# HazyResearch/hyena-dna

Hardware: AMD Instinct MI355X
Metric: nucleotides/sec fwd+bwd at L=1M d=256; fftconv achieved HBM GB/s vs peak (higher is better)
Workload: dtype f32

## Files before the change

### hyena_dna_amd/_lib.py

```python
import ctypes
import os
import threading

import torch

HERE = os.path.dirname(os.path.abspath(__file__))
LIB_PATH = os.path.join(HERE, "csrc", "libhyena_fftconv.so")
ABI_VERSION = 3

HYENA_F32, HYENA_BF16, HYENA_F16 = 0, 1, 2
MAX_L = 1048576
PLAN_NONE, PLAN_ONCHIP, PLAN_TWO_LEVEL = 0, 1, 2

_DTYPES = {torch.float32: HYENA_F32, torch.bfloat16: HYENA_BF16, torch.float16: HYENA_F16}

_lock = threading.Lock()
_lib = None
_tables = {}
_workspace = {}


class HyenaLibraryError(RuntimeError):
    pass

# ... 503 lines not shown
def fftconv_fwd(u, k, bias, chunk=None, save=False, grad=None):
    _require_gpu(u, "u")
    B, D, L = u.shape
    u, k = as_rows(u), as_rows(k)
    ldx, ldk = ld_of(u), ld_of(k)
    out = empty_like_rows(u)
    if B == 0:
        return (out, torch.empty(0, dtype=torch.uint8, device=u.device)) if save else out
    chunk = _chunk_override() if chunk is None else int(chunk)
    tables = tables_for(u.device, L)
    nbytes = lib().hyena_fftconv_workspace_bytes(B, D, L, 0, chunk)
    if (save or torch.is_grad_enabled()) if grad is None else grad:
        nbytes = max(nbytes, lib().hyena_fftconv_workspace_bytes(B, D, L, 1, chunk))
    ws, stream = workspace_for(u.device, nbytes)
    bp = bias.data_ptr() if bias is not None else None
    with _backend.guard(u.device):
        saved = torch.empty(saved_bytes(B, D, L), dtype=torch.uint8, device=u.device) if save else None
        check(lib().hyena_fftconv_fwd_ld(u.data_ptr(), k.data_ptr(), bp, out.data_ptr(), B, D, L, ldx, ldk, dtype_code(u.dtype),
                                         tables.data_ptr(), ws.data_ptr(), ws.numel(), chunk,
                                         saved.data_ptr() if save else None, saved.numel() if save else 0, stream))
    return (out, saved) if save else out


def _same_pitch(t, ld):
    if ld_of(t) == ld:
        return t
    r = empty_rows(t.shape[:-1], t.shape[-1], t.dtype, t.device, pitch=ld)
    r.copy_(t)
    return r


def fftconv_bwd(dout, u, k, bias, need_du=True, need_dk=True, chunk=None, saved=None):
    _require_gpu(dout, "dout")
    B, D, L = dout.shape
    dout = as_rows(dout)
    ldx = ld_of(dout)
    if u is not None:
        u = _same_pitch(as_rows(u), ldx)
    if k is not None:
        k = as_rows(k)
    ldk = ld_of(k) if k is not None else row_pitch(L)
    du = empty_like_rows(dout) if need_du else None
    dk = empty_rows((D,), L, torch.float32, dout.device, pitch=ldk) if need_dk else None
    dbias = torch.empty((D,), dtype=torch.float32, device=dout.device) if need_dk else None
    if B == 0:
        return du, None if dk is None else dk.zero_(), None if dbias is None else dbias.zero_()
    chunk = _chunk_override() if chunk is None else int(chunk)
    tables = tables_for(dout.device, L)
    nbytes = lib().hyena_fftconv_workspace_bytes(B, D, L, 1, chunk)
    ws, stream = workspace_for(dout.device, nbytes)
    bp = bias.data_ptr() if bias is not None else None
    ptr = lambda t: t.data_ptr() if t is not None else None
    with _backend.guard(dout.device):
        check(lib().hyena_fftconv_bwd_ld(dout.data_ptr(), ptr(u), None if saved is not None else ptr(k), bp, ptr(du), ptr(dk), ptr(dbias),
                                         B, D, L, ldx, ldk, dtype_code(dout.dtype), tables.data_ptr(), ws.data_ptr(), ws.numel(),
                                         chunk, ptr(saved), saved.numel() if saved is not None else 0, stream))
    return du, dk, dbias


def mixer_pre_fwd(x, w, b, L):
    _require_gpu(x, "x")
    B, Lx, D3 = x.shape
    D = D3 // 3
    vg = torch.empty((B, D, L), dtype=x.dtype, device=x.device)
    with _backend.guard(x.device):
        check(lib().hyena_mixer_pre_fwd(x.data_ptr(), w.data_ptr(), b.data_ptr(), vg.data_ptr(), B, L, Lx, D,
                                        dtype_code(x.dtype), _backend.stream(x.device)))
    return vg


def mixer_post_fwd(y, x, w, b):
    _require_gpu(x, "x")
    B, D, L = y.shape
    z = torch.empty((B, L, D), dtype=x.dtype, device=x.device)
    with _backend.guard(x.device):
        check(lib().hyena_mixer_post_fwd(y.data_ptr(), x.data_ptr(), w.data_ptr(), b.data_ptr(), z.data_ptr(), B, L,
                                         x.shape[1], D, dtype_code(x.dtype), _backend.stream(x.device)))
    return z


def mixer_partials(x, L):
    B, Lx, D3 = x.shape
    n = lib().hyena_mixer_partial_floats(B, L, D3 // 3)
    return torch.empty(n, dtype=torch.float32, device=x.device).view(B, -1, D3, 4)


def mixer_post_bwd(dz, y, x, w, b, dx, part):
    B, D, L = y.shape
    dy = torch.empty_like(y)
    with _backend.guard(x.device):
        check(lib().hyena_mixer_post_bwd(dz.data_ptr(), y.data_ptr(), x.data_ptr(), w.data_ptr(), b.data_ptr(),
                                         dy.data_ptr(), dx.data_ptr(), part.data_ptr(), B, L, x.shape[1], D,
                                         dtype_code(x.dtype), _backend.stream(x.device)))
    return dy


def mixer_pre_bwd(dvg, x, w, b, dx, part):
    B, D, L = dvg.shape
    with _backend.guard(x.device):
        check(lib().hyena_mixer_pre_bwd(dvg.data_ptr(), x.data_ptr(), w.data_ptr(), b.data_ptr(), dx.data_ptr(),
                                        part.data_ptr(), B, L, x.shape[1], D, dtype_code(x.dtype),
                                        _backend.stream(x.device)))


def cm_pre_fwd(xT, bin_, w, b, L):
    _require_gpu(xT, "xT")
    D3, B, Lx = xT.shape
# ... 643 lines not shown
```

### hyena_dna_amd/csrc/fftconv.hip

```cpp
#include "fftconv_kernels.h"
#include "mixer_kernels.h"
#include "filter_kernels.h"
#include "block_kernels.h"
#include "../../include/hyena_fftconv.h"
#include "../../include/hyena_mixer.h"
#include "../../include/hyena_filter.h"
#include "../../include/hyena_block.h"

#include <cmath>
#include <cstdio>
#include <cstdlib>
#include <vector>

using namespace hyena;

#include "launch.h"
#include "onchip_host.h"

namespace {

struct Plan {
    int L, M, M1;
    int R;
};
// ... 245 lines not shown
        if (hipMemcpyAsync(d_tables, h.data(), h.size() * sizeof(c32), hipMemcpyHostToDevice, (hipStream_t)stream) != hipSuccess)
            return HYENA_ERR_LAUNCH;
        if (hipStreamSynchronize((hipStream_t)stream) != hipSuccess) return HYENA_ERR_LAUNCH;
#endif
        return HYENA_OK;
    }
    const double tau = 6.283185307179586476925286766559;
    for (int i = 0; i < 1024; ++i) {
        double a = -tau * (double)i / (double)p.M;
        h[i].x = (float)std::cos(a);
        h[i].y = (float)std::sin(a);
        double r = -tau * (double)i / 1024.0;
        h[2048 + i].x = (float)std::cos(r);
        h[2048 + i].y = (float)std::sin(r);
    }
    for (int s = 0; s < 32; ++s)
        for (int j = 0; j < 32; ++j) {
            double r = -tau * (double)(s * j) / 1024.0;
            h[3072 + s * 32 + j].x = (float)std::cos(r);
            h[3072 + s * 32 + j].y = (float)std::sin(r);
        }
    for (int i = 0; i < p.M1; ++i) {
        double a = -tau * (double)i / (double)p.M1;
        h[1024 + i].x = (float)std::cos(a);
        h[1024 + i].y = (float)std::sin(a);
    }
#ifdef HIPEMU
    memcpy(d_tables, h.data(), h.size() * sizeof(c32));
#else
    if (hipMemcpyAsync(d_tables, h.data(), h.size() * sizeof(c32), hipMemcpyHostToDevice, (hipStream_t)stream) != hipSuccess)
        return HYENA_ERR_LAUNCH;
    if (hipStreamSynchronize((hipStream_t)stream) != hipSuccess) return HYENA_ERR_LAUNCH;
#endif
    return HYENA_OK;
}

int hyena_fftconv_default_chunk(int B, int D, int L, int backward) {
    Plan p;
    if (!make_plan(L, &p) || B < 1 || D < 1) return 0;
    if (p.R) return D;
    const size_t per_channel = (size_t)(backward ? 2 * B + 2 : B + 1) * p.M * sizeof(c32);
    size_t c = CACHE_BUDGET / per_channel;
    const size_t cmax = ((size_t)1 << 28) / p.M;
    if (c > cmax) c = cmax;
    if (c < 1) c = 1;
    if (c > (size_t)D) c = D;
    return (int)c;
}

size_t hyena_fftconv_workspace_bytes(int B, int D, int L, int backward, int chunk) {
    Plan p;
    if (!make_plan(L, &p) || B < 1 || D < 1) return 0;
    if (p.R)
        return oc::spectrum_bytes(D, p.R) + (backward ? oc::dk_partial_bytes(p.R, B, D, L) + (oc::dk1_ok(p.R, B) ? oc::spectrum_bytes(D, p.R) : 0) : 0);
    if (chunk <= 0) chunk = hyena_fftconv_default_chunk(B, D, L, backward);
    if (chunk > D) chunk = D;
    if ((size_t)chunk * p.M > ((size_t)1 << 28)) chunk = (int)(((size_t)1 << 28) / p.M);
    return (size_t)(backward ? 2 * B + 2 : B + 1) * chunk * p.M * sizeof(c32) +
           (backward ? (size_t)B * chunk * 2 * 1024 * sizeof(c32) : 0);
}

static inline c32* saved_wk(void* saved) { return reinterpret_cast<c32*>(saved); }
static inline c32* saved_wu(void* saved, int D, int M) { return reinterpret_cast<c32*>(saved) + (size_t)D * M; }

size_t hyena_fftconv_saved_bytes(int B, int D, int L) {
    Plan p;
    if (!make_plan(L, &p) || B < 1 || D < 1) return 0;
    if (p.R) return oc::spectrum_bytes(D, p.R);
    return (size_t)(B + 1) * D * p.M * sizeof(c32);
}

static int fwd_impl(const void* u, const float* k, const float* bias, void* out, int B, int D, int L, int ldx, int ldk, int dtype,
                    const void* d_tables, void* workspace, size_t workspace_bytes, int chunk, void* saved,
                    size_t saved_bytes, void* stream) {
    Plan p;
    if (u == nullptr || k == nullptr || out == nullptr || d_tables == nullptr || workspace == nullptr || B < 1 ||
        D < 1 || ldx < L || ldk < L || (dtype != HYENA_F32 && dtype != HYENA_BF16 && dtype != HYENA_F16))
        return HYENA_ERR_BAD_ARG;
    const oc::Pitch ld = {ldx, ldk};
    if (!make_plan(L, &p)) return HYENA_ERR_UNSUPPORTED_L;
    if (p.R) {
        if ((size_t)D * p.M * sizeof(c32) >= ((size_t)1 << 32)) return HYENA_ERR_BAD_ARG;
        if (workspace_bytes < oc::spectrum_bytes(D, p.R)) return HYENA_ERR_WORKSPACE;
        if (saved != nullptr && saved_bytes < oc::spectrum_bytes(D, p.R)) return HYENA_ERR_WORKSPACE;
        if (oc::small_ok(p.R, B, D, L, ld, dtype))
            return oc::launch_small_fwd(p.R, u, out, k, bias, saved, d_tables, B, D, L, ld, dtype, stream);
        void* H = saved ? saved : workspace;
        int st = oc::launch_spec(p.R, k, bias, H, d_tables, D, L, ld, stream);
        if (st) return st;
        return oc::launch_conv(p.R, u, out, H, d_tables, B, D, L, ld, dtype, 0, stream);
    }
    if (chunk <= 0) chunk = hyena_fftconv_default_chunk(B, D, L, 0);
    if (chunk > D) chunk = D;
    if ((size_t)chunk * p.M > ((size_t)1 << 28)) chunk = (int)(((size_t)1 << 28) / p.M);
    if (workspace_bytes < hyena_fftconv_workspace_bytes(B, D, L, 0, chunk)) return HYENA_ERR_WORKSPACE;
    if (saved != nullptr && saved_bytes < hyena_fftconv_saved_bytes(B, D, L)) return HYENA_ERR_WORKSPACE;

    const Tables tab = tables_from(d_tables);
    c32* wsWk = reinterpret_cast<c32*>(workspace);
    c32* wsW = wsWk + (size_t)chunk * p.M;
    const size_t es = elem_size(dtype);
    int st;
    for (int d0 = 0; d0 < D; d0 += chunk) {
        const int cd = (D - d0 < chunk) ? D - d0 : chunk;
        c32* Wk = saved ? saved_wk(saved) + (size_t)d0 * p.M : wsWk;
        c32* Wu = saved ? saved_wu(saved, D, p.M) + (size_t)d0 * p.M : wsW;
        const int ub = saved ? D : cd;
        ColArgs ck;
        ck.x = k + (size_t)d0 * ldk; ck.W = Wk; ck.tab = tab; ck.L = L; ck.inner = cd; ck.w_bstride = cd;
        ck.outer_stride = 0; ck.inner_stride = ldk; ck.aux0 = nullptr; ck.x2 = nullptr; ck.W2 = nullptr;
        if ((st = launch_col<false>(HYENA_F32, p.M1, ck, cd, stream))) return st;
        ColArgs cu;
        cu.x = reinterpret_cast<const char*>(u) + (size_t)d0 * ldx * es; cu.W = Wu; cu.tab = tab; cu.L = L; cu.inner = cd;
        cu.w_bstride = ub;
        cu.outer_stride = (long)D * ldx; cu.inner_stride = ldx; cu.aux0 = nullptr; cu.x2 = nullptr; cu.W2 = nullptr;
        if ((st = launch_col<false>(dtype, p.M1, cu, B * cd, stream))) return st;
        RowArgs rc;
        rc.X = Wu; rc.U = Wk; rc.S = nullptr; rc.S0 = nullptr; rc.bias = bias ? bias + d0 : nullptr; rc.K = nullptr; rc.Y = wsW;
        rc.x_bstride = ub; rc.u_bstride = 0; rc.y_bstride = cd; rc.tab = tab;
        rc.M1 = p.M1; rc.inner = cd; rc.B = B; rc.scale = 1.0f / (float)p.M;
        if ((st = launch_row_prod2<MODE_CONV>(rc, stream))) return st;
        ColArgs co = cu;
        co.x = reinterpret_cast<char*>(out) + (size_t)d0 * ldx * es; co.W = wsW; co.w_bstride = cd;
        if ((st = launch_col<true>(dtype, p.M1, co, B * cd, stream))) return st;
    }
    return HYENA_OK;
}

static int bwd_impl(const void* dout, const void* u, const float* k, const float* bias, void* du, float* dk,
                    float* dbias, int B, int D, int L, int ldx, int ldk, int dtype, const void* d_tables, void* workspace,
                    size_t workspace_bytes, int chunk, const void* saved_c, size_t saved_bytes, void* stream) {
    Plan p;
    void* saved = const_cast<void*>(saved_c);
    const oc::Pitch ld = {ldx, ldk};
    if (dout == nullptr || (u == nullptr && saved == nullptr) || (k == nullptr && saved == nullptr) ||
        d_tables == nullptr || workspace == nullptr || B < 1 || D < 1 || ldx < L || ldk < L ||
        (dtype != HYENA_F32 && dtype != HYENA_BF16 && dtype != HYENA_F16))
        return HYENA_ERR_BAD_ARG;
    if (dbias != nullptr && dk == nullptr) return HYENA_ERR_BAD_ARG;
    if (!make_plan(L, &p)) return HYENA_ERR_UNSUPPORTED_L;
    if (p.R) {
        if (dk != nullptr && u == nullptr) return HYENA_ERR_BAD_ARG;
        if (p.R == 1 && (size_t)B * D * ldx * elem_size(dtype) >= ((size_t)1 << 32)) return HYENA_ERR_BAD_ARG;
        if ((size_t)D * p.M * sizeof(c32) >= ((size_t)1 << 32)) return HYENA_ERR_BAD_ARG;
        if (workspace_bytes < hyena_fftconv_workspace_bytes(B, D, L, 1, chunk)) return HYENA_ERR_WORKSPACE;
        if (saved != nullptr && saved_bytes < oc::spectrum_bytes(D, p.R)) return HYENA_ERR_WORKSPACE;
        void* partials = reinterpret_cast<char*>(workspace) + oc::spectrum_bytes(D, p.R);
        int st;
        if ((du != nullptr || dk != nullptr) && oc::small_ok(p.R, B, D, L, ld, dtype)) {
            const void* H = saved;
            if (H == nullptr) {
                if ((st = oc::launch_small_fwd(p.R, nullptr, nullptr, k, bias, workspace, d_tables, 0, D, L, ld, dtype, stream))) return st;
                H = workspace;
            }
            return oc::launch_small_bwd(p.R, dout, u, du, dk, dbias, H, d_tables, B, D, L, ld, dtype, stream);
        }
        if (du != nullptr) {
            const void* H = saved;
            if (H == nullptr) {
                if ((st = oc::launch_spec(p.R, k, bias, workspace, d_tables, D, L, ld, stream))) return st;
                H = workspace;
            }
            if (dk != nullptr && oc::dkdu_ok(p.R, B))
                return oc::launch_dkdu(p.R, dout, u, du, H, dk, dbias, partials, d_tables, B, D, L, ld, dtype, stream);
            if ((st = oc::launch_conv(p.R, dout, du, H, d_tables, B, D, L, ld, dtype, 1, stream))) return st;
        }
        if (dk != nullptr && oc::dk1_ok(p.R, B)) {
            void* uspec = reinterpret_cast<char*>(partials) + oc::dk_partial_bytes(p.R, B, D, L);
            return oc::launch_dk1(p.R, dout, u, dk, dbias, uspec, d_tables, D, L, ld, dtype, stream);
        }
        if (dk != nullptr && (st = oc::launch_dk(p.R, dout, u, dk, dbias, partials, d_tables, B, D, L, ld, dtype, stream))) return st;
        return HYENA_OK;
    }
    if (chunk <= 0) chunk = hyena_fftconv_default_chunk(B, D, L, 1);
    if (chunk > D) chunk = D;
    if ((size_t)chunk * p.M > ((size_t)1 << 28)) chunk = (int)(((size_t)1 << 28) / p.M);
    if (workspace_bytes < hyena_fftconv_workspace_bytes(B, D, L, 1, chunk)) return HYENA_ERR_WORKSPACE;
    if (saved != nullptr && saved_bytes < hyena_fftconv_saved_bytes(B, D, L)) return HYENA_ERR_WORKSPACE;

    const Tables tab = tables_from(d_tables);
    c32* wsWk = reinterpret_cast<c32*>(workspace);
    c32* Sdk = wsWk + (size_t)chunk * p.M;
    c32* Wg = Sdk + (size_t)chunk * p.M;
    c32* wsWu = Wg + (size_t)B * chunk * p.M;
    c32* S0 = wsWu + (size_t)B * chunk * p.M;
    const size_t es = elem_size(dtype);
    int st;
    for (int d0 = 0; d0 < D; d0 += chunk) {
        const int cd = (D - d0 < chunk) ? D - d0 : chunk;
        c32* Wk = saved ? saved_wk(saved) + (size_t)d0 * p.M : wsWk;
        c32* Wu = saved ? saved_wu(saved, D, p.M) + (size_t)d0 * p.M : wsWu;
        const int ub = saved ? D : cd;
        ColArgs cg;
        cg.x = reinterpret_cast<const char*>(dout) + (size_t)d0 * ldx * es; cg.W = Wg; cg.tab = tab; cg.L = L; cg.inner = cd;
        cg.w_bstride = cd;
        cg.outer_stride = (long)D * ldx; cg.inner_stride = ldx; cg.aux0 = nullptr; cg.x2 = nullptr; cg.W2 = nullptr;
        ColArgs cgu = cg;
        if (dk != nullptr && !saved) { cgu.x2 = reinterpret_cast<const char*>(u) + (size_t)d0 * ldx * es; cgu.W2 = Wu; }
        if ((st = launch_col<false>(dtype, p.M1, cgu, B * cd, stream))) return st;
        ColArgs ck;
        ck.x = saved ? nullptr : k + (size_t)d0 * ldk; ck.W = Wk; ck.tab = tab; ck.L = L; ck.inner = cd; ck.w_bstride = cd;
        ck.outer_stride = 0; ck.inner_stride = ldk; ck.aux0 = nullptr; ck.x2 = nullptr; ck.W2 = nullptr;
        if (du != nullptr && !saved && (st = launch_col<false>(HYENA_F32, p.M1, ck, cd, stream))) return st;
        RowArgs rb;
        rb.X = Wg; rb.U = Wu; rb.S = Sdk; rb.S0 = S0; rb.bias = bias ? bias + d0 : nullptr; rb.K = Wk; rb.Y = Wg;
        rb.x_bstride = cd; rb.u_bstride = ub; rb.y_bstride = cd; rb.tab = tab;
        rb.M1 = p.M1; rb.inner = cd; rb.B = B; rb.scale = 1.0f / (float)p.M;
        if (dk != nullptr) {
            if (du != nullptr) st = launch_row_bwd<true>(rb, stream);
            else st = launch_row_bwd<false>(rb, stream);
            if (st) return st;
            ColArgs cdk;
            cdk.x = dk + (size_t)d0 * ldk; cdk.W = Sdk; cdk.tab = tab; cdk.L = L; cdk.inner = cd; cdk.w_bstride = cd;
            cdk.outer_stride = 0; cdk.inner_stride = ldk; cdk.aux0 = dbias ? dbias + d0 : nullptr; cdk.x2 = nullptr; cdk.W2 = nullptr;
            if ((st = launch_col<true>(HYENA_F32, p.M1, cdk, cd, stream))) return st;
        } else {
// ... 599 lines not shown
```

### hyena_dna_amd/csrc/onchip_dk.hip

```cpp
#define HY_PACKED_F32 1
#ifndef OC_X1_HALVES
#define OC_X1_HALVES 0
#endif
#include <cstdlib>
#include "onchip_kernels.h"
#include "launch.h"
#include "onchip_host.h"
#include "../../include/hyena_fftconv.h"

namespace hyena {
namespace oc {

template <int R, int NP, bool HALF>
static int dk_rh(const DkArgs& a, void* stream) {
    typedef DkCfg<R, NP> K;
    static thread_local int done = -1;
    hy_allow_lds(dk_kernel<R, NP, HALF, 0>, K::LDS, &done);
    HY_LAUNCH((dk_kernel<R, NP, HALF, 0>), dim3(a.D, a.S), dim3(K::WGT), K::LDS, stream, a);
    if constexpr (NP == 2) {
        static thread_local int done1 = -1;
        hy_allow_lds(dk_kernel<R, NP, HALF, 1>, K::LDS, &done1);
        HY_LAUNCH((dk_kernel<R, NP, HALF, 1>), dim3(a.D, a.S), dim3(K::WGT), K::LDS, stream, a);
    }
    if (a.S > 1) HY_LAUNCH((dk_sum_kernel<0>), dim3((a.L + 255) / 256, a.D), dim3(256), 0, stream, a);
    return hy_launch_error() ? HYENA_ERR_LAUNCH : HYENA_OK;
}
template <int R, int NP>
static int dk_r(const DkArgs& a, void* stream) {
    return a.dtype == DT_F32 ? dk_rh<R, NP, false>(a, stream) : dk_rh<R, NP, true>(a, stream);
}
template <int R, bool HALF>
static int dkdu_rh(const DkArgs& a, void* stream) {
    typedef DkCfg<R, 1> K;
    static thread_local int done = -1;
    hy_allow_lds((dk_kernel<R, 1, HALF, 0, true>), K::LDS, &done);
    HY_LAUNCH((dk_kernel<R, 1, HALF, 0, true>), dim3(a.D, a.S), dim3(K::WGT), K::LDS, stream, a);
    if (a.S > 1) HY_LAUNCH((dk_sum_kernel<0>), dim3((a.L + 255) / 256, a.D), dim3(256), 0, stream, a);
    return hy_launch_error() ? HYENA_ERR_LAUNCH : HYENA_OK;
}
template <int R>
static int dkdu_r(const DkArgs& a, void* stream) {
    return a.dtype == DT_F32 ? dkdu_rh<R, false>(a, stream) : dkdu_rh<R, true>(a, stream);
}

template <int R, bool HALF>
static int small_fwd_rh(const SmallFwdArgs& a, void* stream) {
    typedef SmallCfg<R> S;
    static thread_local int done = -1;
    hy_allow_lds(small_fwd_kernel<R, HALF>, S::LDS_FWD, &done);
    HY_LAUNCH((small_fwd_kernel<R, HALF>), dim3(a.D, 1), dim3(S::WGT_FWD), S::LDS_FWD, stream, a);
    return hy_launch_error() ? HYENA_ERR_LAUNCH : HYENA_OK;
}
template <int R, bool HALF>
static int small_bwd_rh(const SmallBwdArgs& a, void* stream) {
    typedef SmallCfg<R> S;
    static thread_local int done = -1;
    hy_allow_lds(small_bwd_kernel<R, HALF>, S::LDS_BWD, &done);
    HY_LAUNCH((small_bwd_kernel<R, HALF>), dim3(a.D), dim3(S::WGT_BWD), S::LDS_BWD, stream, a);
    return hy_launch_error() ? HYENA_ERR_LAUNCH : HYENA_OK;
}
int launch_small_fwd(int R, const void* x, void* out, const float* k, const float* bias, void* Hout, const void* tab, int B, int D, int L,
                     Pitch ld, int dtype, void* stream) {
    SmallFwdArgs a;
    a.x = x; a.out = out; a.k = k; a.bias = bias; a.Hout = reinterpret_cast<c32*>(Hout); a.tab = reinterpret_cast<const c32*>(tab);
    a.B = B; a.D = D; a.L = L; a.dtype = dtype; a.ldx = ld.ldx; a.ldk = ld.ldk;
    const bool half = dtype != DT_F32;
    if (R == 1) return half ? small_fwd_rh<1, true>(a, stream) : small_fwd_rh<1, false>(a, stream);
    if (R == 2) return half ? small_fwd_rh<2, true>(a, stream) : small_fwd_rh<2, false>(a, stream);
    return HYENA_ERR_UNSUPPORTED_L;
}
int launch_small_bwd(int R, const void* dout, const void* u, void* du, float* dk, float* dbias, const void* H, const void* tab, int B, int D,
                     int L, Pitch ld, int dtype, void* stream) {
    SmallBwdArgs a;
    a.dout = dout; a.u = u; a.du = du; a.dk = dk; a.dbias = dbias; a.H = reinterpret_cast<const c32*>(H);
    a.tab = reinterpret_cast<const c32*>(tab); a.B = B; a.D = D; a.L = L; a.dtype = dtype; a.ldx = ld.ldx; a.ldk = ld.ldk;
    const bool half = dtype != DT_F32;
    if (R == 1) return half ? small_bwd_rh<1, true>(a, stream) : small_bwd_rh<1, false>(a, stream);
    if (R == 2) return half ? small_bwd_rh<2, true>(a, stream) : small_bwd_rh<2, false>(a, stream);
    return HYENA_ERR_UNSUPPORTED_L;
}

bool dkdu_ok(int R, int B) {
    const char* e = std::getenv("HYENA_FFTCONV_DUDK");
    if (B < 2 || R < 1 || R > 16) return false;
    if (e != nullptr && e[0] == '0') return false;
    if (e != nullptr && e[0] == '1') return true;
    return R == 16;
}
int launch_dkdu(int R, const void* dout, const void* u, void* du, const void* H, float* dk, float* dbias, void* partials, const void* tab, int B,
                int D, int L, Pitch ld, int dtype, void* stream) {
    DkArgs a;
    a.dout = dout; a.u = u; a.dk = dk; a.dbias = dbias; a.tab = reinterpret_cast<const c32*>(tab);
    a.B = B; a.D = D; a.L = L; a.dtype = dtype; a.ldx = ld.ldx; a.ldk = ld.ldk;
    a.du = du; a.H = reinterpret_cast<const c32*>(H);
    a.S = dk_slices(R, B, D, &a.nb);
    a.part = reinterpret_cast<float*>(partials);
    if (a.S > 1 && partials == nullptr) return HYENA_ERR_WORKSPACE;
#define HY_CALL(r) dkdu_r<r>(a, stream)
    switch (R) {
        case 1: return HY_CALL(1);
        case 2: return HY_CALL(2);
        case 4: return HY_CALL(4);
        case 8: return HY_CALL(8);
        case 16: return HY_CALL(16);
        default: return HYENA_ERR_UNSUPPORTED_L;
    }
#undef HY_CALL
}

int launch_dk(int R, const void* dout, const void* u, float* dk, float* dbias, void* partials, const void* tab, int B, int D, int L,
              Pitch ld, int dtype, void* stream) {
    DkArgs a;
    a.du = nullptr; a.H = nullptr;
    a.dout = dout; a.u = u; a.dk = dk; a.dbias = dbias; a.tab = reinterpret_cast<const c32*>(tab);
    a.B = B; a.D = D; a.L = L; a.dtype = dtype; a.ldx = ld.ldx; a.ldk = ld.ldk;
    a.S = dk_slices(R, B, D, &a.nb);
    a.part = reinterpret_cast<float*>(partials);
    if (a.S > 1 && partials == nullptr) return HYENA_ERR_WORKSPACE;
    if (R == 32) {
        a.tab = reinterpret_cast<const c32*>(tab) + set_entries(32);
        return dk_r<16, 2>(a, stream);
    }
#define HY_CALL(r) dk_r<r, 1>(a, stream)
    switch (R) {
        case 1: return HY_CALL(1);
        case 2: return HY_CALL(2);
        case 4: return HY_CALL(4);
        case 8: return HY_CALL(8);
        case 16: return HY_CALL(16);
        default: return HYENA_ERR_UNSUPPORTED_L;
    }
#undef HY_CALL
}

}
}
```

### hyena_dna_amd/csrc/onchip_host.h

```cpp
#pragma once
#include <stddef.h>

namespace hyena {
namespace oc {

enum { MAX_L = 32768 };

struct Pitch { int ldx, ldk; };

int plan_r(int L);
size_t table_entries(int R);
size_t set_entries(int R);
void build_tables(int R, float* host_c32);
size_t spectrum_bytes(int D, int R);

int launch_spec(int R, const float* k, const float* bias, void* H, const void* tab, int D, int L, Pitch ld, void* stream);
int launch_conv(int R, const void* x, void* out, const void* H, const void* tab, int B, int D, int L, Pitch ld, int dtype, int conj,
                void* stream);
size_t dk_partial_bytes(int R, int B, int D, int L);
int dk_slices(int R, int B, int D, int* nb_out);
int launch_dk(int R, const void* dout, const void* u, float* dk, float* dbias, void* partials, const void* tab, int B, int D, int L,
              Pitch ld, int dtype, void* stream);

bool dkdu_ok(int R, int B);
int launch_dkdu(int R, const void* dout, const void* u, void* du, const void* H, float* dk, float* dbias, void* partials, const void* tab, int B,
                int D, int L, Pitch ld, int dtype, void* stream);

bool dk1_ok(int R, int B);
int launch_dk1(int R, const void* dout, const void* u, float* dk, float* dbias, void* Uspec, const void* tab, int D, int L, Pitch ld,
               int dtype, void* stream);

bool small_ok(int R, int B, int D, int L, Pitch ld, int dtype);
int launch_small_fwd(int R, const void* x, void* out, const float* k, const float* bias, void* Hout, const void* tab, int B, int D, int L,
                     Pitch ld, int dtype, void* stream);
int launch_small_bwd(int R, const void* dout, const void* u, void* du, float* dk, float* dbias, const void* H, const void* tab, int B, int D,
                     int L, Pitch ld, int dtype, void* stream);

}
}
```

### hyena_dna_amd/csrc/onchip_kernels.h

```cpp
#pragma once
#define HY_HELPERS_ONLY
#include "fftconv_kernels.h"

namespace hyena {
namespace oc {

#ifdef HIPEMU
#define HY_WAVE_SYNC() hipemu::yield(2)
#else
#define HY_WAVE_SYNC() __builtin_amdgcn_wave_barrier()
#endif

#if defined(OC_PROFILE) && !defined(HIPEMU)
__device__ unsigned long long* oc_prof_buf = nullptr;
struct Prof { unsigned long long t[32]; };
#define OC_MARK(c, i)                                                                                               \
    do {                                                                                                            \
        __builtin_amdgcn_sched_barrier(0);                                                                          \
        if ((c).prof != nullptr) asm volatile("s_memtime %0\n\ts_waitcnt lgkmcnt(0)" : "=s"((c).prof->t[i])::"memory"); \
        __builtin_amdgcn_sched_barrier(0);                                                                          \
    } while (0)
#else
#define OC_MARK(c, i) do {} while (0)
#endif
// ... 392 lines not shown
#ifdef HIPEMU
    HY_UNROLL
    for (int s = 0; s < 32; ++s) {
        const int n = tid + T * s;
        if (n < L) io_st<HALF>(ob, row_off + (unsigned)n * ES, y[s], bf);
    }
#else
    unsigned vo = row_off + (unsigned)tid * ES;
#ifdef OC_DBG_NO_IO
    float acc = 0.f;
    HY_UNROLL
    for (int s = 0; s < 32; ++s) acc += y[s];
    io_st<HALF>(ob, vo, acc, bf);
#else
    HY_UNROLL
    for (int s = 0; s < 32; ++s) {
        if (!PRED || tid + T * s < L) io_st<HALF>(ob, vo, y[s], bf);
        vo += (unsigned)T * ES;
        HY_OPAQUE(vo);
    }
#endif
#endif
}

struct SpecArgs {
    const void* k;
    const float* bias;
    c32* H;
    const c32* tab;
    int D, L, dtype;
    int ld;
};
struct ConvArgs {
    const void* x;
    void* out;
    const c32* H;
    const c32* tab;
    int B, D, L, dtype;
    float conj_sign;
    int ldx, ldo;
};
struct DkArgs {
    const void* dout;
    const void* u;
    float* dk;
    float* dbias;
    const c32* tab;
    float* part;
    int B, D, L, dtype;
    int S, nb;
    int ldx, ldk;
    void* du;
    const c32* H;
};

#ifndef OC_MINW
#define OC_MINW 4
#endif

template <int R> struct WgCfg {
    static constexpr int T = Cfg<R>::T;
    static constexpr int WGT = T < 64 ? 64 : T;
    static constexpr int RPW = WGT / T;
    static constexpr size_t LDS = Cfg<R>::XBYTES * RPW;
};

template <int R>
__device__ __forceinline__ Ctx make_ctx(HY_LDS char* smem, int rg, int tid, const c32* tab) {
    Ctx c;
    c.xb = smem + (size_t)rg * Cfg<R>::XBYTES;
    c.tab = make_gbuf(tab, (unsigned)Cfg<R>::TWN * 8u);
    c.tid = tid;
    c.ka = tid / R;
    c.tp = tid % R;
#if defined(OC_PROFILE) && !defined(HIPEMU)
    c.prof = nullptr;
#endif
    return c;
}

template <int R, bool HALF = false>
__global__ void __launch_bounds__(WgCfg<R>::WGT, OC_MINW) spec_kernel(SpecArgs a) {
    typedef Cfg<R> C;
    constexpr int T = C::T, RPW = WgCfg<R>::RPW;
    constexpr unsigned ES = HALF ? 2u : 4u;
    HY_SMEM(smem);
    const bool bf = a.dtype == DT_BF16;
    const int rg = RPW == 1 ? 0 : (int)threadIdx.x / T, tid = RPW == 1 ? (int)threadIdx.x : (int)threadIdx.x % T;
    const int d0 = blockIdx.x * RPW;
    const int d_raw = d0 + rg;
    const bool valid = d_raw < a.D;
    const int d = valid ? d_raw : a.D - 1;
    const Ctx c = make_ctx<R>(HY_LDS_CAST(char, smem), rg, tid, a.tab);
    const int nrows = (a.D - d0) < RPW ? (a.D - d0) : RPW;
    const GBuf kb = make_gbuf(reinterpret_cast<const char*>(a.k) + (size_t)d0 * a.ld * ES, ((unsigned)(nrows - 1) * (unsigned)a.ld + (unsigned)a.L) * ES);
    c32 v[32];
    load_row<R, 2, HALF, (RPW > 1)>(v, kb, bf, tid, (unsigned)(d - d0) * (unsigned)a.ld * ES, a.L);
    fft_fwd<R>(v, c);
    const float bias = (a.bias != nullptr) ? a.bias[d] : 0.f;
    const float sc = 1.0f / (float)C::M;
    if (valid) {
        c32* Hd = a.H + (size_t)d * C::M + tid;
        HY_UNROLL
        for (int q = 0; q < 32; ++q) Hd[q * T] = mk((v[q].x + bias) * sc, v[q].y * sc);
    }
}
// ... 72 lines not shown
    asm volatile("s_memrealtime %0\n\ts_waitcnt lgkmcnt(0)" : "=s"(rt1)::"memory");
    if (oc_prof_buf != nullptr && (threadIdx.x & 63) == 0) {
        unsigned long long* o = oc_prof_buf + ((size_t)blockIdx.x * (WgCfg<R>::WGT / 64) + (threadIdx.x >> 6)) * 32;
        HY_UNROLL
        for (int i = 0; i < 25; ++i) o[i] = prof.t[i];
        unsigned hw, xcc;
        asm volatile("s_getreg_b32 %0, hwreg(HW_REG_HW_ID)" : "=s"(hw));
        asm volatile("s_getreg_b32 %0, hwreg(HW_REG_XCC_ID)" : "=s"(xcc));
        o[25] = ((unsigned long long)xcc << 32) | hw;
        o[26] = rt0;
        o[27] = rt1;
    }
#endif
}

template <int UNUSED = 0>
__global__ void __launch_bounds__(256) dk_bias_kernel(const float* dk, float* dbias, int D, int ld) {
    const int d = (int)(blockIdx.x * 256 + threadIdx.x);
    if (d < D) dbias[d] = dk[(size_t)d * ld];
}

template <int R, int NP> struct DkCfg {
    static constexpr int T = Cfg<R>::T;
    static constexpr int BP = (512 / T > 16) ? 16 : 512 / T;
    static constexpr int WGT = T * BP;
    static_assert(WGT == 512 && (NP == 1 || BP == 1), "dk workgroups are 512 threads");
    static constexpr size_t LDS_X = Cfg<R>::XBYTES * BP;
    static constexpr size_t LDS_RED = BP > 1 ? (size_t)BP * Cfg<R>::M * 8 : 0;
    static constexpr int PARKQ = NP == 2 ? 16 : 0;
    static constexpr size_t PARK = (size_t)PARKQ * WGT * 8;
    static constexpr size_t LDS = (LDS_X > LDS_RED ? LDS_X : LDS_RED) + PARK;
};

template <int R, int NP, bool HALF, int PHI8>
__device__ __forceinline__ void dk_load(c32 (&v)[32], GBuf xb, bool bf, int tid, unsigned row_off, int L, float sigma) {
    if constexpr (NP == 1) {
        load_row<R, PHI8, HALF, (Cfg<R>::T < 64)>(v, xb, bf, tid, row_off, L);
    } else {
        constexpr int T = Cfg<R>::T, MS = Cfg<R>::M;
        const float r = 0.70710678118654752440f * sigma;
        float xa[32], xc[32];
        load_raw<T, HALF, false>(xa, xb, bf, tid, 0u, L, 0);
        load_raw<T, HALF, false>(xc, xb, bf, tid, 0u, L, MS);
        HY_UNROLL
        for (int s = 0; s < 32; ++s) {
            const c32 y = mk(xa[s] + r * xc[s], -r * xc[s]);
            v[s] = cmul(y, twist_const<PHI8>(s));
        }
    }
}

template <int R, int NP, bool HALF, int E0, bool DU = false>
__global__ void __launch_bounds__((DkCfg<R, NP>::WGT)) dk_kernel(DkArgs a) {
    static_assert(!DU || NP == 1, "du rides on dk only where the row is one transform (M <= 16384)");
    typedef Cfg<R> C;
    typedef DkCfg<R, NP> K;
    constexpr int T = C::T, BP = K::BP;
    constexpr unsigned ES = HALF ? 2u : 4u;
    HY_SMEM(smem);
    const bool bf = a.dtype == DT_BF16;
    const int rg = BP == 1 ? 0 : (int)threadIdx.x / T, tid = BP == 1 ? (int)threadIdx.x : (int)threadIdx.x % T;
    const int d = blockIdx.x;
    const int sl = blockIdx.y;
    const int b_lo = sl * a.nb, b_hi = (b_lo + a.nb < a.B) ? b_lo + a.nb : a.B;
    const bool sliced = a.S > 1;
    Ctx c = make_ctx<R>(HY_LDS_CAST(char, smem), rg, tid, a.tab);
    const unsigned rowbytes = (unsigned)a.L * ES;
    const float sc = 1.0f / (float)(C::M * NP);
    float* dkrow = sliced ? a.part + ((size_t)sl * a.D + d) * a.L : a.dk + (size_t)d * a.ldk;
    float* dbias = sliced ? nullptr : a.dbias;
    {
        constexpr int e = E0;
        constexpr int PHI_A = NP == 2 ? 1 : 2, PHI_B = 5;
        const float sigma = e ? -1.f : 1.f;
        if constexpr (NP == 2) c.tab = make_gbuf(a.tab + e * C::TWN, (unsigned)C::TWN * 8u);
        c32 acc[32];
        HY_UNROLL
        for (int q = 0; q < 32; ++q) acc[q] = mk(0.f, 0.f);
        constexpr int NREG = 32 - K::PARKQ;
        HY_LDS lc32* const park = HY_LDS_CAST(lc32, HY_LDS_CAST(char, smem) + (K::LDS - K::PARK)) + threadIdx.x;
        HY_UNROLL
        for (int q = NREG; q < 32; ++q) lds_st(park + (q - NREG) * K::WGT, mk(0.f, 0.f));
        for (int b0 = b_lo; b0 < b_hi; b0 += BP) {
            const bool live = b0 + rg < b_hi;
            const int b = live ? b0 + rg : b_hi - 1;
            const size_t row = ((size_t)b * a.D + d) * a.ldx * ES;
            constexpr bool WHOLE = T < 64;
            const unsigned whole = (unsigned)((((size_t)a.B * a.D - 1) * a.ldx + a.L) * ES);
            const GBuf gb = WHOLE ? make_gbuf(a.dout, whole) : make_gbuf(reinterpret_cast<const char*>(a.dout) + row, rowbytes);
            const GBuf ub = WHOLE ? make_gbuf(a.u, whole) : make_gbuf(reinterpret_cast<const char*>(a.u) + row, rowbytes);
            const unsigned row_off = WHOLE ? (unsigned)row : 0u;
            c32 u[32], v[32];
            if (e == 0) dk_load<R, NP, HALF, PHI_A>(u, ub, bf, tid, row_off, a.L, sigma);
            else dk_load<R, NP, HALF, PHI_B>(u, ub, bf, tid, row_off, a.L, sigma);
            fft_fwd<R, true>(u, c);
            HY_SCHED_FENCE();
            if (e == 0) dk_load<R, NP, HALF, PHI_A>(v, gb, bf, tid, row_off, a.L, sigma);
            else dk_load<R, NP, HALF, PHI_B>(v, gb, bf, tid, row_off, a.L, sigma);
            fft_fwd<R, true>(v, c);
            HY_SCHED_FENCE();
            const float lv = live ? 1.f : 0.f;
            HY_UNROLL
            for (int q = 0; q < 32; ++q) {
                const c32 p = cmulc(v[q], u[q]);
                if (q < NREG) acc[q] = mk(acc[q].x + lv * p.x, acc[q].y + lv * p.y);
                else {
                    const c32 o = lds_ld(park + (q - NREG) * K::WGT);
                    lds_st(park + (q - NREG) * K::WGT, mk(o.x + lv * p.x, o.y + lv * p.y));
                }
            }
            if constexpr (DU) {
                HY_SCHED_FENCE();
                const GBuf hb = make_gbuf(a.H, (unsigned)a.D * (unsigned)C::M * 8u);
                const unsigned ho = ((unsigned)d * (unsigned)C::M + (unsigned)tid) * 8u;
                HY_UNROLL
                for (int q0 = 0; q0 < 32; q0 += 8) {
                    c32 h[8];
                    HY_UNROLL
                    for (int q = 0; q < 8; ++q) h[q] = gb_ld(hb, ho, (unsigned)((q0 + q) * T) * 8u);
                    HY_UNROLL
                    for (int q = 0; q < 8; ++q) v[q0 + q] = cmul(v[q0 + q], mk(h[q].x, -h[q].y));
                    HY_SCHED_FENCE();
                }
                fft_inv<R>(v, c);
                float y[32];
                HY_UNROLL
                for (int s = 0; s < 32; ++s) {
                    const c32 w = twist_const<2>(s);
                    y[s] = v[s].x * w.x + v[s].y * w.y;
                }
                const GBuf ob = WHOLE ? make_gbuf(a.du, whole) : make_gbuf(reinterpret_cast<char*>(a.du) + row, live ? rowbytes : 0u);
                store_row<T, HALF, WHOLE>(ob, bf, tid, row_off, live ? a.L : 0, y);
                HY_SCHED_FENCE();
            }
        }
        HY_UNROLL
        for (int q = NREG; q < 32; ++q) acc[q] = lds_ld(park + (q - NREG) * K::WGT);
        if constexpr (BP > 1) {
            __syncthreads();
            HY_LDS lc32* red = HY_LDS_CAST(lc32, smem);
            if (rg > 0) {
                HY_UNROLL
                for (int q = 0; q < 32; ++q) lds_st(red + rg * C::M + q * T + tid, acc[q]);
            }
            __syncthreads();
            if (rg == 0) {
                const int ng = (b_hi - b_lo) < BP ? (b_hi - b_lo) : BP;
                for (int o = 1; o < ng; ++o) {
                    HY_UNROLL
                    for (int q = 0; q < 32; ++q) acc[q] = cadd(acc[q], lds_ld(red + o * C::M + q * T + tid));
                }
            }
            __syncthreads();
        }
        fft_inv<R>(acc, c);
        if (rg == 0) {
            if constexpr (NP == 1) {
                HY_UNROLL
                for (int s = 0; s < 32; ++s) {
                    const c32 w = twist_const<2>(s);
                    const int n = tid + T * s;
                    const float val = (acc[s].x * w.x + acc[s].y * w.y) * sc;
                    if (n < a.L) dkrow[n] = val;
                    if (n == 0 && dbias != nullptr) dbias[d] = val;
                }
            } else {
                const float rr = 0.70710678118654752440f;
                HY_UNROLL
                for (int s = 0; s < 32; ++s) {
                    const c32 h = cmulc(acc[s], e ? twist_const<PHI_B>(s) : twist_const<PHI_A>(s));
                    const int n = tid + T * s;
                    const float lo = h.x * sc, hi = (h.x - h.y) * rr * sc;
                    if (e == 0) {
                        if (n < a.L) dkrow[n] = lo;
                        if (n + C::M < a.L) dkrow[n + C::M] = hi;
                    } else {
                        if (n < a.L) {
                            const float val = dkrow[n] + lo;
                            dkrow[n] = val;
                            if (n == 0 && dbias != nullptr) dbias[d] = val;
                        }
                        if (n + C::M < a.L) dkrow[n + C::M] -= hi;
                    }
                }
            }
        }
    }
}

template <int UNUSED = 0>
__global__ void __launch_bounds__(256) dk_sum_kernel(DkArgs a) {
    const int d = blockIdx.y;
    const int n = (int)(blockIdx.x * 256 + threadIdx.x);
    if (n >= a.L) return;
    float acc = a.part[(size_t)d * a.L + n];
    for (int s = 1; s < a.S; ++s) acc += a.part[((size_t)s * a.D + d) * a.L + n];
    a.dk[(size_t)d * a.ldk + n] = acc;
    if (n == 0 && a.dbias != nullptr) a.dbias[d] = acc;
}


struct SmallFwdArgs {
    const void* x;
    void* out;
    const float* k;
    const float* bias;
    c32* Hout;
    const c32* tab;
    int B, D, L, dtype;
    int ldx, ldk;
};
struct SmallBwdArgs {
    const void* dout;
    const void* u;
    void* du;
    float* dk;
    float* dbias;
    const c32* H;
    const c32* tab;
    int B, D, L, dtype;
    int ldx, ldk;
};

template <int R> struct SmallCfg {
    static_assert(R <= 2, "row groups must not contain workgroup barriers");
    static constexpr int T = Cfg<R>::T;
    static constexpr int G = 256 / T;
    static constexpr int FG = 64 / T;
    static constexpr int WGT_FWD = 256 + 64;
    static constexpr int WGT_BWD = 512;
    static constexpr size_t LDS_XF = Cfg<R>::XBYTES * (G + FG);
    static constexpr size_t LDS_FWD = LDS_XF + (size_t)Cfg<R>::M * 8;
    static constexpr size_t LDS_XB = Cfg<R>::XBYTES * 2 * G;
    static constexpr size_t LDS_BWD = LDS_XB + (size_t)G * Cfg<R>::M * 8;
};

template <int R, bool HALF>
__global__ void __launch_bounds__(SmallCfg<R>::WGT_FWD) small_fwd_kernel(SmallFwdArgs a) {
    typedef Cfg<R> C;
    typedef SmallCfg<R> S;
// ... 166 lines not shown
```

Before: 169.5 million.

## Fuse du computation into dk kernel for R=32 using split half-spectra

For the R=32 on-chip plan, the backward pass now computes du alongside dk inside the two-pass dk kernel (NP=2) instead of running a separate spectrum and convolution pass. A new hpar kernel builds the two twisted half-spectra of the filter from k and bias. The dk kernel multiplies the already-transformed dout by those spectra, inverse-transforms, and combines the two halves through a per-row float scratch buffer. This avoids re-reading and re-transforming dout for du, at the cost of extra scratch traffic, a larger workspace, and higher register pressure. The Python side now always passes k, so the filter spectrum is rebuilt even when a saved spectrum exists.

Result: no change. 169.5 million, median of 2 (+0.1%).

```diff
diff --git a/hyena_dna_amd/_lib.py b/hyena_dna_amd/_lib.py
--- a/hyena_dna_amd/_lib.py
+++ b/hyena_dna_amd/_lib.py
@@ -579,7 +579,7 @@
     bp = bias.data_ptr() if bias is not None else None
     ptr = lambda t: t.data_ptr() if t is not None else None
     with _backend.guard(dout.device):
-        check(lib().hyena_fftconv_bwd_ld(dout.data_ptr(), ptr(u), None if saved is not None else ptr(k), bp, ptr(du), ptr(dk), ptr(dbias),
+        check(lib().hyena_fftconv_bwd_ld(dout.data_ptr(), ptr(u), ptr(k), bp, ptr(du), ptr(dk), ptr(dbias),
                                          B, D, L, ldx, ldk, dtype_code(dout.dtype), tables.data_ptr(), ws.data_ptr(), ws.numel(),
                                          chunk, ptr(saved), saved.numel() if saved is not None else 0, stream))
     return du, dk, dbias
diff --git a/hyena_dna_amd/csrc/fftconv.hip b/hyena_dna_amd/csrc/fftconv.hip
--- a/hyena_dna_amd/csrc/fftconv.hip
+++ b/hyena_dna_amd/csrc/fftconv.hip
@@ -321,7 +321,8 @@
     Plan p;
     if (!make_plan(L, &p) || B < 1 || D < 1) return 0;
     if (p.R)
-        return oc::spectrum_bytes(D, p.R) + (backward ? oc::dk_partial_bytes(p.R, B, D, L) + (oc::dk1_ok(p.R, B) ? oc::spectrum_bytes(D, p.R) : 0) : 0);
+        return oc::spectrum_bytes(D, p.R) + (backward ? oc::dk_partial_bytes(p.R, B, D, L) + (oc::dk1_ok(p.R, B) ? oc::spectrum_bytes(D, p.R) : 0) +
+                                                            oc::dkdu_scratch_bytes(p.R, B, D) : 0);
     if (chunk <= 0) chunk = hyena_fftconv_default_chunk(B, D, L, backward);
     if (chunk > D) chunk = D;
     if ((size_t)chunk * p.M > ((size_t)1 << 28)) chunk = (int)(((size_t)1 << 28) / p.M);
@@ -424,13 +425,17 @@
             }
             return oc::launch_small_bwd(p.R, dout, u, du, dk, dbias, H, d_tables, B, D, L, ld, dtype, stream);
         }
+        if (du != nullptr && dk != nullptr && p.R == 32 && k != nullptr && du != dout && oc::dkdu_ok(p.R, B)) {
+            void* scratch = reinterpret_cast<char*>(partials) + oc::dk_partial_bytes(p.R, B, D, L);
+            return oc::launch_dkdu(p.R, dout, u, du, nullptr, dk, dbias, partials, d_tables, B, D, L, ld, dtype, stream, k, bias, workspace, scratch);
+        }
         if (du != nullptr) {
             const void* H = saved;
             if (H == nullptr) {
                 if ((st = oc::launch_spec(p.R, k, bias, workspace, d_tables, D, L, ld, stream))) return st;
                 H = workspace;
             }
-            if (dk != nullptr && oc::dkdu_ok(p.R, B))
+            if (dk != nullptr && p.R <= 16 && oc::dkdu_ok(p.R, B))
                 return oc::launch_dkdu(p.R, dout, u, du, H, dk, dbias, partials, d_tables, B, D, L, ld, dtype, stream);
             if ((st = oc::launch_conv(p.R, dout, du, H, d_tables, B, D, L, ld, dtype, 1, stream))) return st;
         }
diff --git a/hyena_dna_amd/csrc/onchip_dk.hip b/hyena_dna_amd/csrc/onchip_dk.hip
--- a/hyena_dna_amd/csrc/onchip_dk.hip
+++ b/hyena_dna_amd/csrc/onchip_dk.hip
@@ -42,6 +42,19 @@
 static int dkdu_r(const DkArgs& a, void* stream) {
     return a.dtype == DT_F32 ? dkdu_rh<R, false>(a, stream) : dkdu_rh<R, true>(a, stream);
 }
+template <bool HALF>
+static int dkdu32_h(const DkArgs& a, const HparArgs& h, void* stream) {
+    typedef DkCfg<16, 2> K;
+    static thread_local int doneh = -1, done0 = -1, done1 = -1;
+    hy_allow_lds(hpar_kernel<0>, Cfg<16>::XBYTES, &doneh);
+    HY_LAUNCH((hpar_kernel<0>), dim3(h.D, 2), dim3(512), Cfg<16>::XBYTES, stream, h);
+    hy_allow_lds((dk_kernel<16, 2, HALF, 0, true>), K::LDS, &done0);
+    HY_LAUNCH((dk_kernel<16, 2, HALF, 0, true>), dim3(a.D, a.S), dim3(K::WGT), K::LDS, stream, a);
+    hy_allow_lds((dk_kernel<16, 2, HALF, 1, true>), K::LDS, &done1);
+    HY_LAUNCH((dk_kernel<16, 2, HALF, 1, true>), dim3(a.D, a.S), dim3(K::WGT), K::LDS, stream, a);
+    if (a.S > 1) HY_LAUNCH((dk_sum_kernel<0>), dim3((a.L + 255) / 256, a.D), dim3(256), 0, stream, a);
+    return hy_launch_error() ? HYENA_ERR_LAUNCH : HYENA_OK;
+}
 
 template <int R, bool HALF>
 static int small_fwd_rh(const SmallFwdArgs& a, void* stream) {
@@ -82,20 +95,30 @@
 
 bool dkdu_ok(int R, int B) {
     const char* e = std::getenv("HYENA_FFTCONV_DUDK");
-    if (B < 2 || R < 1 || R > 16) return false;
+    if (B < 2 || R < 1 || R > 32) return false;
     if (e != nullptr && e[0] == '0') return false;
     if (e != nullptr && e[0] == '1') return true;
     return R == 16;
 }
+size_t dkdu_scratch_bytes(int R, int B, int D) { return R == 32 && dkdu_ok(R, B) ? (size_t)B * D * 32768 * sizeof(float) : 0; }
 int launch_dkdu(int R, const void* dout, const void* u, void* du, const void* H, float* dk, float* dbias, void* partials, const void* tab, int B,
-                int D, int L, Pitch ld, int dtype, void* stream) {
+                int D, int L, Pitch ld, int dtype, void* stream, const float* k, const float* bias, void* hpar, void* scratch) {
     DkArgs a;
+    a.Hpar = nullptr; a.scr = nullptr;
     a.dout = dout; a.u = u; a.dk = dk; a.dbias = dbias; a.tab = reinterpret_cast<const c32*>(tab);
     a.B = B; a.D = D; a.L = L; a.dtype = dtype; a.ldx = ld.ldx; a.ldk = ld.ldk;
     a.du = du; a.H = reinterpret_cast<const c32*>(H);
     a.S = dk_slices(R, B, D, &a.nb);
     a.part = reinterpret_cast<float*>(partials);
     if (a.S > 1 && partials == nullptr) return HYENA_ERR_WORKSPACE;
+    if (R == 32) {
+        if (k == nullptr || hpar == nullptr || scratch == nullptr) return HYENA_ERR_BAD_ARG;
+        a.tab = reinterpret_cast<const c32*>(tab) + set_entries(32);
+        a.Hpar = reinterpret_cast<const c32*>(hpar); a.scr = reinterpret_cast<float*>(scratch);
+        HparArgs h;
+        h.k = k; h.bias = bias; h.Hpar = reinterpret_cast<c32*>(hpar); h.tab = a.tab; h.D = D; h.L = L; h.ldk = ld.ldk;
+        return dtype == DT_F32 ? dkdu32_h<false>(a, h, stream) : dkdu32_h<true>(a, h, stream);
+    }
 #define HY_CALL(r) dkdu_r<r>(a, stream)
     switch (R) {
         case 1: return HY_CALL(1);
@@ -111,7 +134,7 @@
 int launch_dk(int R, const void* dout, const void* u, float* dk, float* dbias, void* partials, const void* tab, int B, int D, int L,
               Pitch ld, int dtype, void* stream) {
     DkArgs a;
-    a.du = nullptr; a.H = nullptr;
+    a.du = nullptr; a.H = nullptr; a.Hpar = nullptr; a.scr = nullptr;
     a.dout = dout; a.u = u; a.dk = dk; a.dbias = dbias; a.tab = reinterpret_cast<const c32*>(tab);
     a.B = B; a.D = D; a.L = L; a.dtype = dtype; a.ldx = ld.ldx; a.ldk = ld.ldk;
     a.S = dk_slices(R, B, D, &a.nb);
diff --git a/hyena_dna_amd/csrc/onchip_host.h b/hyena_dna_amd/csrc/onchip_host.h
--- a/hyena_dna_amd/csrc/onchip_host.h
+++ b/hyena_dna_amd/csrc/onchip_host.h
@@ -23,8 +23,10 @@
               Pitch ld, int dtype, void* stream);
 
 bool dkdu_ok(int R, int B);
+size_t dkdu_scratch_bytes(int R, int B, int D);
 int launch_dkdu(int R, const void* dout, const void* u, void* du, const void* H, float* dk, float* dbias, void* partials, const void* tab, int B,
-                int D, int L, Pitch ld, int dtype, void* stream);
+                int D, int L, Pitch ld, int dtype, void* stream, const float* k = nullptr, const float* bias = nullptr, void* hpar = nullptr,
+                void* scratch = nullptr);
 
 bool dk1_ok(int R, int B);
 int launch_dk1(int R, const void* dout, const void* u, float* dk, float* dbias, void* Uspec, const void* tab, int D, int L, Pitch ld,
diff --git a/hyena_dna_amd/csrc/onchip_kernels.h b/hyena_dna_amd/csrc/onchip_kernels.h
--- a/hyena_dna_amd/csrc/onchip_kernels.h
+++ b/hyena_dna_amd/csrc/onchip_kernels.h
@@ -468,6 +468,8 @@
     int ldx, ldk;
     void* du;
     const c32* H;
+    const c32* Hpar;
+    float* scr;
 };
 
 #ifndef OC_MINW
@@ -646,7 +648,6 @@
 
 template <int R, int NP, bool HALF, int E0, bool DU = false>
 __global__ void __launch_bounds__((DkCfg<R, NP>::WGT)) dk_kernel(DkArgs a) {
-    static_assert(!DU || NP == 1, "du rides on dk only where the row is one transform (M <= 16384)");
     typedef Cfg<R> C;
     typedef DkCfg<R, NP> K;
     constexpr int T = C::T, BP = K::BP;
@@ -694,8 +695,19 @@
             fft_fwd<R, true>(v, c);
             HY_SCHED_FENCE();
             const float lv = live ? 1.f : 0.f;
+            c32 hh[(DU && NP == 2) ? 32 : 1];
             HY_UNROLL
             for (int q = 0; q < 32; ++q) {
+                if constexpr (DU && NP == 2) {
+                    if (q == NREG) {
+                        HY_SCHED_FENCE();
+                        const GBuf hb = make_gbuf(a.Hpar + (size_t)e * a.D * C::M, (unsigned)a.D * (unsigned)C::M * 8u);
+                        const unsigned ho = ((unsigned)d * (unsigned)C::M + (unsigned)tid) * 8u;
+                        HY_UNROLL
+                        for (int h = 0; h < 32; ++h) hh[h] = gb_ld(hb, ho, (unsigned)(h * T) * 8u);
+                        HY_SCHED_FENCE();
+                    }
+                }
                 const c32 p = cmulc(v[q], u[q]);
                 if (q < NREG) acc[q] = mk(acc[q].x + lv * p.x, acc[q].y + lv * p.y);
                 else {
@@ -703,7 +715,44 @@
                     lds_st(park + (q - NREG) * K::WGT, mk(o.x + lv * p.x, o.y + lv * p.y));
                 }
             }
-            if constexpr (DU) {
+            if constexpr (DU && NP == 2) {
+                HY_SCHED_FENCE();
+                HY_UNROLL
+                for (int q = 0; q < 32; ++q) v[q] = cmul(v[q], mk(hh[q].x, -hh[q].y));
+                HY_SCHED_FENCE();
+                const GBuf sb = make_gbuf(a.scr + ((size_t)b * a.D + d) * (size_t)(2 * C::M), (unsigned)(2 * C::M) * 4u);
+                float p[32], p2[32];
+                if (e == 1) {
+                    load_raw<T, false, false>(p, sb, false, tid, 0u, 2 * C::M, 0);
+                    HY_SCHED_FENCE();
+                }
+                fft_inv<R>(v, c);
+                if (e == 1) {
+                    load_raw<T, false, false>(p2, sb, false, tid, 0u, 2 * C::M, C::M);
+                    HY_SCHED_FENCE();
+                }
+                const float rr = 0.70710678118654752440f;
+                float lo[32], hi[32];
+                HY_UNROLL
+                for (int s = 0; s < 32; ++s) {
+                    const c32 w = e ? twist_const<PHI_B>(s) : twist_const<PHI_A>(s);
+                    lo[s] = v[s].x * w.x + v[s].y * w.y;
+                    hi[s] = v[s].x * ((w.x + w.y) * rr) + v[s].y * ((w.y - w.x) * rr);
+                }
+                if (e == 0) {
+                    store_row<T, false, false>(sb, false, tid, 0u, C::M, lo);
+                    store_row<T, false, false>(sb, false, tid, (unsigned)C::M * 4u, C::M, hi);
+                } else {
+                    HY_UNROLL
+                    for (int s = 0; s < 32; ++s) lo[s] = p[s] + lo[s];
+                    const GBuf ob = make_gbuf(reinterpret_cast<char*>(a.du) + row, live ? rowbytes : 0u);
+                    store_row<T, HALF, false>(ob, bf, tid, 0u, live ? a.L : 0, lo);
+                    HY_UNROLL
+                    for (int s = 0; s < 32; ++s) hi[s] = p2[s] - hi[s];
+                    store_row<T, HALF, false>(ob, bf, tid, (unsigned)C::M * ES, live ? a.L - C::M : 0, hi);
+                }
+                HY_SCHED_FENCE();
+            } else if constexpr (DU) {
                 HY_SCHED_FENCE();
                 const GBuf hb = make_gbuf(a.H, (unsigned)a.D * (unsigned)C::M * 8u);
                 const unsigned ho = ((unsigned)d * (unsigned)C::M + (unsigned)tid) * 8u;
@@ -780,6 +829,32 @@
             }
         }
     }
+}
+
+struct HparArgs {
+    const float* k;
+    const float* bias;
+    c32* Hpar;
+    const c32* tab;
+    int D, L, ldk;
+};
+template <int UNUSED = 0>
+__global__ void __launch_bounds__(512) hpar_kernel(HparArgs a) {
+    typedef Cfg<16> C;
+    constexpr int T = C::T;
+    HY_SMEM(smem);
+    const int tid = (int)threadIdx.x, d = blockIdx.x, e = blockIdx.y;
+    const Ctx c = make_ctx<16>(HY_LDS_CAST(char, smem), 0, tid, a.tab + e * C::TWN);
+    const GBuf kb = make_gbuf(a.k + (size_t)d * a.ldk, (unsigned)a.L * 4u);
+    c32 v[32];
+    if (e == 0) dk_load<16, 2, false, 1>(v, kb, false, tid, 0u, a.L, 1.f);
+    else dk_load<16, 2, false, 5>(v, kb, false, tid, 0u, a.L, -1.f);
+    fft_fwd<16>(v, c);
+    const float bias = (a.bias != nullptr) ? a.bias[d] : 0.f;
+    const float sc = 1.0f / (float)(2 * C::M);
+    c32* Hd = a.Hpar + ((size_t)e * a.D + d) * C::M + tid;
+    HY_UNROLL
+    for (int q = 0; q < 32; ++q) Hd[q * T] = mk((v[q].x + bias) * sc, v[q].y * sc);
 }
 
 template <int UNUSED = 0>
```
